# rskew/aiko_services

Measured on AMD Instinct MI355X. Metric: frames/sec (whole node) + p50 latency, ResNet-50 pipeline at 1/2/4/8 MI355X, higher is better.
Workload: dtype bf16; 1 GPU; global_batch=640, per_gpu_batch=640, parallelism=dp1, hipgraph=True, ingest=hbm, setup_frames=12, model=resnet50, pipeline=(SyntheticFrames ResNet50Classifier ClassifierTopK), gpu_lanes=2

## Files before the change

### aiko_services_amd/csrc/kernels/bneck_fused.hip

```cpp
#include <cstdlib>
#include <type_traits>

#include "conv_common.h"

namespace aiko {

namespace {

constexpr int kBnW = 56;
constexpr int kBnMid = 64;
constexpr int kBnOut = 256;
constexpr int kBnNW = 8;
constexpr int kBnTPW = 2;
constexpr int kBnTU = 8 * 64 + 8;
constexpr int kBnTB = kBnTU * 16;

struct BnParams {
  const bf16_t* x;
  const bf16_t* w1;
  const float* b1;
  const bf16_t* w2;
  const float* b2;
  const bf16_t* w3;
  const float* b3;
  bf16_t* y;
  int B, H;
  int rows_per_wg, rows_rem;
  unsigned* dbg;
  int mode;
};

__device__ __forceinline__ void bn_barrier() {
  asm volatile("s_waitcnt lgkmcnt(0)\n\ts_barrier" ::: "memory");
}

__device__ __forceinline__ void bn_vm_wait(int n) {
  switch (n) {
#define BN_W(k) case k: asm volatile("s_waitcnt vmcnt(" #k ")" ::: "memory"); break;
    BN_W(1) BN_W(2) BN_W(3) BN_W(4) BN_W(5) BN_W(6) BN_W(7) BN_W(8) BN_W(9) BN_W(10) BN_W(11) BN_W(12)
    BN_W(13) BN_W(14) BN_W(15) BN_W(16) BN_W(17) BN_W(18) BN_W(19) BN_W(20) BN_W(21) BN_W(22) BN_W(23)
    BN_W(24) BN_W(25) BN_W(26) BN_W(27) BN_W(28)
#undef BN_W
    default: asm volatile("s_waitcnt vmcnt(0)" ::: "memory"); break;
  }
}

template <int KS, int R, int D>
__device__ __forceinline__ void bn_pipeline() {
  __builtin_amdgcn_sched_group_barrier(0x100, R * D, 0);
#pragma unroll
  for (int k = 0; k < KS - D; ++k) {
    __builtin_amdgcn_sched_group_barrier(0x008, R, 0);
    __builtin_amdgcn_sched_group_barrier(0x100, R, 0);
  }
  __builtin_amdgcn_sched_group_barrier(0x008, R * D, 0);
}

__device__ __forceinline__ void bn_store16(bf16_t* p, u32x4 v) {
  asm volatile("global_store_dwordx4 %0, %1, off\n\ts_nop 1" :: "v"(p), "v"(v) : "memory");
}

template <int OFF>
__device__ __forceinline__ bf16x8 bn_ld(const unsigned char* base) {
  return *reinterpret_cast<const bf16x8*>(base + OFF);
}

__device__ __forceinline__ uint32_t bn_relu2(uint32_t v) {
  typedef short s16x2 __attribute__((ext_vector_type(2)));
  const s16x2 r = __builtin_elementwise_max(__builtin_bit_cast(s16x2, v), s16x2{0, 0});
  return __builtin_bit_cast(uint32_t, r);
}

template <int CIN>
__global__ __launch_bounds__(64 * kBnNW, 1) void bneck_fused_kernel(BnParams p) {
  constexpr bool DUAL = CIN == 64;
  constexpr int NC = CIN / 8;
  constexpr int XPU = NC + 2;
  constexpr int XU = kBnW * XPU;
  constexpr int XB = XU * 16;
  constexpr int NI = (XU + 63) / 64;
  constexpr int DQ = (NI + kBnNW - 1) / kBnNW;
  constexpr int KS1 = CIN / 32, KS2 = 9 * kBnMid / 32, K3 = DUAL ? 2 * kBnMid : kBnMid, KS3 = K3 / 32;
  constexpr int ST = 2 * kBnTPW;
  constexpr int X_BYTES = 4 * XB, T1_BYTES = 3 * kBnTB;
  constexpr int LDS_BYTES = X_BYTES + T1_BYTES + kBnTB;
  static_assert(LDS_BYTES <= 160 * 1024, "LDS");
  __shared__ __attribute__((aligned(16))) unsigned char lds[LDS_BYTES];
  unsigned char* const xr = lds;
  unsigned char* const t1r = lds + X_BYTES;
  unsigned char* const t2b = lds + X_BYTES + T1_BYTES;

  const int tid = threadIdx.x, lane = tid & 63;
  const int wv = __builtin_amdgcn_readfirstlane(tid >> 6);
  const int cg = wv & 3;
  const int pt0 = (wv >> 2) * kBnTPW;
  const int fr = lane & 15, fq = lane >> 4;

  const int lid = xcd_remap(blockIdx.x, gridDim.x);
  const int H = p.H, HV = H + 2;
  const int R0 = lid * p.rows_per_wg + min(lid, p.rows_rem);
  const int nrows = p.rows_per_wg + (lid < p.rows_rem ? 1 : 0);
  if (nrows <= 0) return;
  const int n0 = R0 / H, h0 = R0 - n0 * H;

  bf16x8 w1f[KS1], w2f[KS2], w3f[4][KS3];
#pragma unroll
  for (int ks = 0; ks < KS1; ++ks)
    w1f[ks] = *reinterpret_cast<const bf16x8*>(p.w1 + (16 * cg + fr) * CIN + 32 * ks + 8 * fq);
#pragma unroll
  for (int ks = 0; ks < KS2; ++ks)
    w2f[ks] = *reinterpret_cast<const bf16x8*>(p.w2 + (16 * cg + fr) * (9 * kBnMid) + 32 * ks + 8 * fq);
#pragma unroll
  for (int t = 0; t < 4; ++t) {
    const int row = 64 * cg + 32 * (t >> 1) + 8 * (fr >> 2) + 4 * (t & 1) + (fr & 3);
#pragma unroll
    for (int ks = 0; ks < KS3; ++ks)
      w3f[t][ks] = *reinterpret_cast<const bf16x8*>(p.w3 + row * K3 + 32 * ks + 8 * fq);
  }
  f32x4 bias1, bias2;
#pragma unroll
  for (int e = 0; e < 4; ++e) {
    bias1[e] = p.b1[16 * cg + 4 * fq + e];
    bias2[e] = p.b2[16 * cg + 4 * fq + e];
  }
  f32x4 bias3[4];
#pragma unroll
  for (int t = 0; t < 4; ++t)
#pragma unroll
    for (int e = 0; e < 4; ++e) bias3[t][e] = p.b3[64 * cg + 32 * (t >> 1) + 8 * fq + 4 * (t & 1) + e];
  bf16x8 eye[2];
#pragma unroll
  for (int tp = 0; tp < 2; ++tp)
#pragma unroll
    for (int i = 0; i < 8; ++i)
      eye[tp][i] = (fq == (fr >> 2) && i == 4 * tp + (fr & 3)) ? (bf16_t)1.0f : (bf16_t)0.0f;
  if (tid < 3) *reinterpret_cast<u32x4*>(t1r + tid * kBnTB) = u32x4{0u, 0u, 0u, 0u};
  __builtin_amdgcn_s_waitcnt(0x0f70);

  int goff[DQ];
  bool gok[DQ];
#pragma unroll
  for (int q = 0; q < DQ; ++q) {
    const int u = (wv + kBnNW * q) * 64 + lane;
    const int s = min(u / XPU, kBnW - 1);
    const int c = min(u - (u / XPU) * XPU, NC - 1);
    goff[q] = s * CIN * 2 + c * 16;
    gok[q] = u < XU && wv + kBnNW * q < NI && u - (u / XPU) * XPU < NC;
  }
  int dw = 0;
#pragma unroll
  for (int q = 0; q < DQ; ++q) dw += wv + kBnNW * q < NI ? 1 : 0;

  const int xlb = ((16 * pt0 + fr) * XPU + fq) * 16;
  const int tlb = (fq * 64 + fr + 16 * pt0) * 16;
  const int twb = ((2 * cg + (fq >> 1)) * 64 + fr + 16 * pt0) * 16 + (fq & 1) * 8;

  constexpr long XROWG = (long)kBnW * CIN * 2;
  const int nl = (R0 + nrows - 1) / H;
  const int vlast = (nl - n0) * HV + (R0 + nrows - 1 - nl * H) + 2;
  int ops = 0;
  unsigned long long marks = 0;
  int vdma = h0, dn = n0, dr = h0 - 1;
  auto dma_next = [&]() {
    const int v = vdma++;
    int m = -1;
    if (dr >= 0 && dr < H) {
      const unsigned char* src = reinterpret_cast<const unsigned char*>(p.x) + ((long)dn * H + dr) * XROWG;
      unsigned char* dst = xr + (v & 3) * XB;
#pragma unroll
      for (int q = 0; q < DQ; ++q) {
        const int j = wv + kBnNW * q;
        if (gok[q]) glds16_asm(src + goff[q], dst + j * 1024);
      }
      ops += dw;
      m = ops;
    }
    if (++dr > H) {
      dr = -1;
      ++dn;
    }
    marks = (marks << 16) | (m >= 0 ? 0x8000ull | (unsigned)(m & 0x7fff) : 0ull);
  };
  auto slot_mark = [&](int v) {
    return (unsigned)(marks >> (16 * (vdma - 1 - v))) & 0xffffu;
  };
  auto row_valid = [&](int v) { return (slot_mark(v) & 0x8000u) != 0; };
  auto wait_row = [&](int v) {
    const unsigned mk = slot_mark(v);
    if (mk & 0x8000u) bn_vm_wait(__builtin_amdgcn_readfirstlane((int)(((unsigned)ops - mk) & 0x7fffu)));
  };

  auto conv1 = [&](int k) {
    unsigned char* t1w = t1r + (k % 3) * kBnTB + twb;
    if (!row_valid(k)) {
#pragma unroll
      for (int t = 0; t < kBnTPW; ++t) *reinterpret_cast<uint2*>(t1w + (1 + 16 * t) * 16) = uint2{0u, 0u};
      return;
    }
    const unsigned char* xs = xr + (k & 3) * XB + xlb;
    f32x4 a1[kBnTPW];
#pragma unroll
    for (int ks = 0; ks < KS1; ++ks) {
      bf16x8 bf[kBnTPW];
#pragma unroll
      for (int t = 0; t < kBnTPW; ++t)
        bf[t] = *reinterpret_cast<const bf16x8*>(xs + (16 * t * XPU + 4 * ks) * 16);
#pragma unroll
      for (int t = 0; t < kBnTPW; ++t)
        a1[t] = __builtin_amdgcn_mfma_f32_16x16x32_bf16(w1f[ks], bf[t], ks == 0 ? bias1 : a1[t], 0, 0, 0);
    }
    bn_pipeline<KS1, kBnTPW, KS1 >= 4 ? 3 : 1>();
#pragma unroll
    for (int t = 0; t < kBnTPW; ++t) {
      uint2 pk{bn_relu2(pack2(a1[t][0], a1[t][1])), bn_relu2(pack2(a1[t][2], a1[t][3]))};
      if (pt0 + t == 3 && fr >= kBnW - 48) pk = uint2{0u, 0u};
      *reinterpret_cast<uint2*>(t1w + (1 + 16 * t) * 16) = pk;
    }
  };

  f32x4 a2n[kBnTPW];
  auto conv2_part = [&](int vc, auto kb, auto ke) __attribute__((always_inline)) {
    constexpr int KB = decltype(kb)::value, KE = decltype(ke)::value;
    const unsigned char* tr[3] = {t1r + ((vc - 1) % 3) * kBnTB + tlb, t1r + (vc % 3) * kBnTB + tlb,
                                  t1r + ((vc + 1) % 3) * kBnTB + tlb};
#pragma unroll
    for (int ks = KB; ks < KE; ++ks) {
      const int tap = ks >> 1, dy = tap / 3, dx = tap % 3 - 1, hk = ks & 1;
      bf16x8 bf[kBnTPW];
#pragma unroll
      for (int t = 0; t < kBnTPW; ++t)
        bf[t] = *reinterpret_cast<const bf16x8*>(tr[dy] + (1 + 256 * hk + 16 * t + dx) * 16);
#pragma unroll
      for (int t = 0; t < kBnTPW; ++t)
        a2n[t] = __builtin_amdgcn_mfma_f32_16x16x32_bf16(w2f[ks], bf[t], ks == 0 ? bias2 : a2n[t], 0, 0, 0);
    }
    bn_pipeline<KE - KB, kBnTPW, 4>();
  };
  auto conv2_store = [&]() __attribute__((always_inline)) {
    unsigned char* t2w = t2b + twb;
#pragma unroll
    for (int t = 0; t < kBnTPW; ++t) {
      const uint2 pk{bn_relu2(pack2(a2n[t][0], a2n[t][1])), bn_relu2(pack2(a2n[t][2], a2n[t][3]))};
      *reinterpret_cast<uint2*>(t2w + (1 + 16 * t) * 16) = pk;
    }
  };
  using KB0 = std::integral_constant<int, 0>;
  using KBS = std::integral_constant<int, 12>;
  using KBE = std::integral_constant<int, KS2>;

  auto conv3 = [&](int vc, int n, int r) {
    const unsigned char* xres = xr + (vc & 3) * XB + xlb;
    const unsigned char* t2r = t2b + tlb;
    bf16_t* yrow = p.y + ((long)(n * H + r) * kBnW + 16 * pt0 + fr) * kBnOut + 64 * cg + 8 * fq;
#pragma unroll
    for (int t8 = 0; t8 < kBnTPW; ++t8) {
      bf16x8 bf[KS3];
#pragma unroll
      for (int ks = 0; ks < KS3; ++ks)
        bf[ks] = ks < 2 ? *reinterpret_cast<const bf16x8*>(t2r + (1 + 256 * ks + 16 * t8) * 16)
                        : *reinterpret_cast<const bf16x8*>(xres + (16 * t8 * XPU + 4 * (ks - 2)) * 16);
      bf16x8 rv[2];
      if constexpr (!DUAL) {
#pragma unroll
        for (int h = 0; h < 2; ++h)
          rv[h] = *reinterpret_cast<const bf16x8*>(xres + (16 * t8 * XPU + 8 * cg + 4 * h) * 16);
      }
      f32x4 a3[4];
#pragma unroll
      for (int ks = 0; ks < KS3; ++ks)
#pragma unroll
        for (int t = 0; t < 4; ++t)
          a3[t] = __builtin_amdgcn_mfma_f32_16x16x32_bf16(w3f[t][ks], bf[ks], ks == 0 ? bias3[t] : a3[t], 0, 0, 0);
      if constexpr (!DUAL) {
#pragma unroll
        for (int t = 0; t < 4; ++t) a3[t] = __builtin_amdgcn_mfma_f32_16x16x32_bf16(eye[t & 1], rv[t >> 1], a3[t], 0, 0, 0);
      }
#pragma unroll
      for (int h = 0; h < 2; ++h) {
        const u32x4 ov{bn_relu2(pack2(a3[2 * h][0], a3[2 * h][1])), bn_relu2(pack2(a3[2 * h][2], a3[2 * h][3])),
                       bn_relu2(pack2(a3[2 * h + 1][0], a3[2 * h + 1][1])),
                       bn_relu2(pack2(a3[2 * h + 1][2], a3[2 * h + 1][3]))};
        if (p.mode & 128) {
          if (ov[0] == 0x7fc07fc0u && ov[1] == ov[2] && ov[3] == 1u) bn_store16(yrow, ov);
        } else if (p.mode & 256) {
          bf16_t* yr = p.y + ((long)(n * H + r) * kBnW) * kBnOut;
          bn_store16(yr + (long)(((cg * 2 + (pt0 >> 1)) * 4 + t8 * 2 + h) % 28) * 512 + lane * 8, ov);
        } else if (16 * (pt0 + t8) + fr < kBnW) {
          bn_store16(yrow + 16 * t8 * kBnOut + 32 * h, ov);
        }
      }
    }
    ops += ST;
  };

  while (vdma <= min(h0 + 3, vlast)) dma_next();
  wait_row(min(h0 + 2, vlast));
  wait_row(h0 + 1);
  wait_row(h0);
  bn_barrier();
  conv1(h0);
  conv1(h0 + 1);
  if (h0 + 2 <= vlast) conv1(h0 + 2);
  bn_barrier();

  int n = n0, r = h0, vc = h0 + 1;
  const bool stamps = p.dbg != nullptr && wv == 0;
  unsigned st[8];
  bool pre = false;
  auto stamp = [&](int i) {
    if (stamps) st[i] = (unsigned)__builtin_amdgcn_s_memtime();
  };
  for (int j = 0; j < nrows; ++j) {
    stamp(0);
    if (j > 0) {
      if (++r == H) {
        r = 0;
        ++n;
        vc += 3;
      } else {
        ++vc;
      }
    }
    while (!(p.mode & 32) && vdma <= min(vc + 3, vlast)) dma_next();
    stamp(1);
    if (j > 0 && r == 0) {
      wait_row(vc + 1);
      wait_row(vc);
      bn_barrier();
      conv1(vc);
      conv1(vc + 1);
      bn_barrier();
    }
    if (!(p.mode & 1)) {
      if (pre) conv2_part(vc, KBS{}, KBE{});
      else conv2_part(vc, KB0{}, KBE{});
      conv2_store();
    }
    stamp(2);
    if (!(p.mode & 8) && vc + 2 <= vlast) wait_row(vc + 2);
    stamp(3);
    if (!(p.mode & 16)) bn_barrier();
    stamp(4);
    const bool split = (p.mode & 3072) && j + 1 < nrows && r + 1 < H;
    if (split && (p.mode & 2048)) conv2_part(vc + 1, KB0{}, KBS{});
    if (p.mode & 512) {
      if (!(p.mode & 4)) conv3(vc, n, r);
      stamp(5);
      if (!(p.mode & 2) && vc + 2 <= vlast) conv1(vc + 2);
    } else {
      if (!(p.mode & 2) && vc + 2 <= vlast) conv1(vc + 2);
      stamp(5);
      if (!(p.mode & 4)) conv3(vc, n, r);
    }
    if (split && !(p.mode & 2048)) conv2_part(vc + 1, KB0{}, KBS{});
    pre = split;
    stamp(6);
    if (!(p.mode & 16)) bn_barrier();
    stamp(7);
    if (stamps) {
      unsigned* d = p.dbg + ((long)lid * (p.rows_per_wg + 1) + j) * 8;
      if (lane == 0) {
        bn_store16(reinterpret_cast<bf16_t*>(d), u32x4{st[0], st[1], st[2], st[3]});
        bn_store16(reinterpret_cast<bf16_t*>(d + 4), u32x4{st[4], st[5], st[6], st[7]});
      }
      ops += 2;
    }
  }
  asm volatile("s_waitcnt vmcnt(0)" ::: "memory");
}

}

}

static int bn_cu_count() {
  static int n = 0;
  if (n == 0) {
    int dev = 0;
    if (hipGetDevice(&dev) != hipSuccess ||
        hipDeviceGetAttribute(&n, hipDeviceAttributeMultiprocessorCount, dev) != hipSuccess || n <= 0)
      n = 256;
  }
  return n;
}

extern "C" int aiko_bneck_fused(const void* x, const void* w1, const float* b1, const void* w2, const float* b2,
                                const void* w3, const float* b3, void* y, int B, int H, int W, int cin, int grid,
                                unsigned* dbg, hipStream_t stream) {
  using namespace aiko;
  if (W != kBnW || (cin != 64 && cin != 256) || B <= 0 || H <= 0) return -1;
  const int R = B * H;
  int G = grid > 0 ? grid : bn_cu_count();
  G = G < R ? G : R;
  BnParams p;
  p.x = static_cast<const bf16_t*>(x);
  p.w1 = static_cast<const bf16_t*>(w1);
  p.b1 = b1;
  p.w2 = static_cast<const bf16_t*>(w2);
  p.b2 = b2;
  p.w3 = static_cast<const bf16_t*>(w3);
  p.b3 = b3;
  p.y = static_cast<bf16_t*>(y);
  p.B = B;
  p.H = H;
  p.rows_per_wg = R / G;
  p.rows_rem = R % G;
  p.dbg = dbg;
  const char* mode = getenv("AIKO_BN_MODE");
  p.mode = mode ? atoi(mode) : 1024;
  if (cin == 256)
    hipLaunchKernelGGL(bneck_fused_kernel<256>, dim3(G), dim3(64 * kBnNW), 0, stream, p);
  else
    hipLaunchKernelGGL(bneck_fused_kernel<64>, dim3(G), dim3(64 * kBnNW), 0, stream, p);
  return (int)hipGetLastError();
}
```

Before: 98750 frames/s.

## Add lean bottleneck kernel path with rotating LDS buffers and specialized interior rows

Adds a LEAN template variant of the fused bottleneck kernel, enabled by default unless debug stamps or a non-default mode are set. It uses rotating LDS slot offsets for the input and conv1 rows, and asm helpers for global-to-LDS DMA and stores with immediate offsets. It also splits the per-row loop into a boundary path and a stripped-down interior path, and overlaps the next row's conv2 prefix with the current row. The aim is to cut per-row index arithmetic, branching and waits in the inner pipeline. In exchange it adds a second large code path whose boundary handling must be exactly right.

```diff
diff --git a/aiko_services_amd/csrc/kernels/bneck_fused.hip b/aiko_services_amd/csrc/kernels/bneck_fused.hip
--- a/aiko_services_amd/csrc/kernels/bneck_fused.hip
+++ b/aiko_services_amd/csrc/kernels/bneck_fused.hip
@@ -60,6 +60,19 @@
   asm volatile("global_store_dwordx4 %0, %1, off\n\ts_nop 1" :: "v"(p), "v"(v) : "memory");
 }
 
+template <bool HALF>
+__device__ __forceinline__ void bn_store16_row(const unsigned char* row, uint32_t off, u32x4 v) {
+  if constexpr (HALF)
+    asm volatile("global_store_dwordx4 %0, %1, off offset:64\n\ts_nop 1" :: "v"(row + off), "v"(v) : "memory");
+  else
+    asm volatile("global_store_dwordx4 %0, %1, off\n\ts_nop 1" :: "v"(row + off), "v"(v) : "memory");
+}
+
+__device__ __forceinline__ void bn_glds16_row(const unsigned char* row, uint32_t off, uint32_t m0v) {
+  asm volatile("s_mov_b32 m0, %1\n\ts_nop 0\n\tglobal_load_lds_dwordx4 %0, off"
+               :: "v"(row + off), "s"(m0v) : "memory", "m0");
+}
+
 template <int OFF>
 __device__ __forceinline__ bf16x8 bn_ld(const unsigned char* base) {
   return *reinterpret_cast<const bf16x8*>(base + OFF);
@@ -71,7 +84,7 @@
   return __builtin_bit_cast(uint32_t, r);
 }
 
-template <int CIN>
+template <int CIN, bool LEAN>
 __global__ __launch_bounds__(64 * kBnNW, 1) void bneck_fused_kernel(BnParams p) {
   constexpr bool DUAL = CIN == 64;
   constexpr int NC = CIN / 8;
@@ -292,6 +305,197 @@
     }
     ops += ST;
   };
+
+  if constexpr (LEAN) {
+    static_assert(ST + DQ <= 28, "bn_vm_wait");
+    const int Rend = R0 + nrows;
+    const int nle = (Rend - 1) / H, hle = Rend - 1 - nle * H;
+    const int F0 = h0 > 0 ? R0 - 1 : R0;
+    const int F1 = hle + 1 < H ? Rend : Rend - 1;
+    const unsigned char* const xg = reinterpret_cast<const unsigned char*>(p.x);
+    const uint32_t xm0 = __builtin_amdgcn_readfirstlane(static_cast<uint32_t>(reinterpret_cast<uintptr_t>(xr))) +
+                         wv * 1024;
+    auto dma_row = [&](const unsigned char* src, uint32_t slot) {
+#pragma unroll
+      for (int q = 0; q < DQ; ++q)
+        if (gok[q]) bn_glds16_row(src, (uint32_t)goff[q], xm0 + slot + q * (kBnNW * 1024));
+    };
+    auto wait_dma = [&]() {
+      if (dw == DQ) bn_vm_wait(ST + DQ);
+      else bn_vm_wait(ST + DQ - 1);
+    };
+    auto conv1_x = [&](uint32_t xo, uint32_t to) {
+      unsigned char* t1w = t1r + to + twb;
+      const unsigned char* xs = xr + xo + xlb;
+      f32x4 a1[kBnTPW];
+#pragma unroll
+      for (int ks = 0; ks < KS1; ++ks) {
+        bf16x8 bf[kBnTPW];
+#pragma unroll
+        for (int t = 0; t < kBnTPW; ++t)
+          bf[t] = *reinterpret_cast<const bf16x8*>(xs + (16 * t * XPU + 4 * ks) * 16);
+#pragma unroll
+        for (int t = 0; t < kBnTPW; ++t)
+          a1[t] = __builtin_amdgcn_mfma_f32_16x16x32_bf16(w1f[ks], bf[t], ks == 0 ? bias1 : a1[t], 0, 0, 0);
+      }
+      bn_pipeline<KS1, kBnTPW, KS1 >= 4 ? 3 : 1>();
+#pragma unroll
+      for (int t = 0; t < kBnTPW; ++t) {
+        uint2 pk{bn_relu2(pack2(a1[t][0], a1[t][1])), bn_relu2(pack2(a1[t][2], a1[t][3]))};
+        if (pt0 + t == 3 && fr >= kBnW - 48) pk = uint2{0u, 0u};
+        *reinterpret_cast<uint2*>(t1w + (1 + 16 * t) * 16) = pk;
+      }
+    };
+    auto conv1_zero = [&](uint32_t to) {
+      unsigned char* t1w = t1r + to + twb;
+#pragma unroll
+      for (int t = 0; t < kBnTPW; ++t) *reinterpret_cast<uint2*>(t1w + (1 + 16 * t) * 16) = uint2{0u, 0u};
+    };
+    auto conv2_rows = [&](uint32_t o0, uint32_t o1, uint32_t o2, auto kb, auto ke) __attribute__((always_inline)) {
+      constexpr int KB = decltype(kb)::value, KE = decltype(ke)::value;
+      const unsigned char* tr[3] = {t1r + o0 + tlb, t1r + o1 + tlb, t1r + o2 + tlb};
+#pragma unroll
+      for (int ks = KB; ks < KE; ++ks) {
+        const int tap = ks >> 1, dy = tap / 3, dx = tap % 3 - 1, hk = ks & 1;
+        bf16x8 bf[kBnTPW];
+#pragma unroll
+        for (int t = 0; t < kBnTPW; ++t)
+          bf[t] = *reinterpret_cast<const bf16x8*>(tr[dy] + (1 + 256 * hk + 16 * t + dx) * 16);
+#pragma unroll
+        for (int t = 0; t < kBnTPW; ++t)
+          a2n[t] = __builtin_amdgcn_mfma_f32_16x16x32_bf16(w2f[ks], bf[t], ks == 0 ? bias2 : a2n[t], 0, 0, 0);
+      }
+      bn_pipeline<KE - KB, kBnTPW, 4>();
+    };
+    const uint32_t yoff = ((16 * pt0 + fr) * kBnOut + 64 * cg + 8 * fq) * 2;
+    auto conv3_row = [&](uint32_t xo, const unsigned char* yrow) {
+      const unsigned char* xres = xr + xo + xlb;
+      const unsigned char* t2r = t2b + tlb;
+#pragma unroll
+      for (int t8 = 0; t8 < kBnTPW; ++t8) {
+        bf16x8 bf[KS3];
+#pragma unroll
+        for (int ks = 0; ks < KS3; ++ks)
+          bf[ks] = ks < 2 ? *reinterpret_cast<const bf16x8*>(t2r + (1 + 256 * ks + 16 * t8) * 16)
+                          : *reinterpret_cast<const bf16x8*>(xres + (16 * t8 * XPU + 4 * (ks - 2)) * 16);
+        bf16x8 rv[2];
+        if constexpr (!DUAL) {
+#pragma unroll
+          for (int h = 0; h < 2; ++h)
+            rv[h] = *reinterpret_cast<const bf16x8*>(xres + (16 * t8 * XPU + 8 * cg + 4 * h) * 16);
+        }
+        f32x4 a3[4];
+#pragma unroll
+        for (int ks = 0; ks < KS3; ++ks)
+#pragma unroll
+          for (int t = 0; t < 4; ++t)
+            a3[t] = __builtin_amdgcn_mfma_f32_16x16x32_bf16(w3f[t][ks], bf[ks], ks == 0 ? bias3[t] : a3[t], 0, 0, 0);
+        if constexpr (!DUAL) {
+#pragma unroll
+          for (int t = 0; t < 4; ++t) a3[t] = __builtin_amdgcn_mfma_f32_16x16x32_bf16(eye[t & 1], rv[t >> 1], a3[t], 0, 0, 0);
+        }
+        const uint32_t yo = yoff + t8 * (16 * kBnOut * 2);
+        const bool live = 16 * (pt0 + t8) + fr < kBnW;
+        const u32x4 o0{bn_relu2(pack2(a3[0][0], a3[0][1])), bn_relu2(pack2(a3[0][2], a3[0][3])),
+                       bn_relu2(pack2(a3[1][0], a3[1][1])), bn_relu2(pack2(a3[1][2], a3[1][3]))};
+        if (live) bn_store16_row<false>(yrow, yo, o0);
+        const u32x4 o1{bn_relu2(pack2(a3[2][0], a3[2][1])), bn_relu2(pack2(a3[2][2], a3[2][3])),
+                       bn_relu2(pack2(a3[3][0], a3[3][1])), bn_relu2(pack2(a3[3][2], a3[3][3]))};
+        if (live) bn_store16_row<true>(yrow, yo, o1);
+      }
+    };
+
+    const uint32_t s0 = h0 > 0 ? 1u : 0u;
+    uint32_t X0 = s0 * XB, X1 = (s0 + 1) * XB, X2 = (s0 + 2) * XB, X3 = ((s0 + 3) & 3u) * XB;
+    uint32_t T0 = 0, T1 = kBnTB, T2 = 2 * kBnTB;
+    int f = R0;
+    const unsigned char* src = xg + (long)(R0 + 3) * XROWG;
+    const unsigned char* yp = reinterpret_cast<const unsigned char*>(p.y) + (long)R0 * (kBnW * kBnOut * 2);
+    bool pre = false;
+    auto advance = [&]() {
+      ++f;
+      src += XROWG;
+      yp += kBnW * kBnOut * 2;
+      const uint32_t x0 = X0;
+      X0 = X1, X1 = X2, X2 = X3, X3 = x0;
+    };
+    auto rotate_t1 = [&]() {
+      const uint32_t t0 = T0;
+      T0 = T1, T1 = T2, T2 = t0;
+    };
+
+    auto row_general = [&](int r, int rb, int xe, bool boundary) {
+      const bool dma = f + 3 <= F1;
+      if (dma) dma_row(src, X3);
+      if (boundary) {
+        conv1_x(X0, T1);
+        if (1 <= xe) conv1_x(X1, T2);
+        else conv1_zero(T2);
+        bn_barrier();
+      }
+      if (pre) conv2_rows(T0, T1, T2, KBS{}, KBE{});
+      else conv2_rows(T0, T1, T2, KB0{}, KBE{});
+      conv2_store();
+      if (dma) wait_dma();
+      else bn_vm_wait(ST);
+      bn_barrier();
+      if (r + 2 <= xe) conv1_x(X2, T0);
+      else conv1_zero(T0);
+      conv3_row(X0, yp);
+      pre = r + 1 < rb;
+      if (pre) {
+        rotate_t1();
+        conv2_rows(T0, T1, T2, KB0{}, KBS{});
+      }
+      bn_barrier();
+      advance();
+    };
+    auto row_interior = [&]() {
+      dma_row(src, X3);
+      conv2_rows(T0, T1, T2, KBS{}, KBE{});
+      conv2_store();
+      wait_dma();
+      bn_barrier();
+      conv1_x(X2, T0);
+      conv3_row(X0, yp);
+      rotate_t1();
+      conv2_rows(T0, T1, T2, KB0{}, KBS{});
+      bn_barrier();
+      advance();
+    };
+
+    int r = h0, rem = nrows;
+    {
+      const unsigned char* s = xg + (long)F0 * XROWG;
+      const int npro = min(R0 + 2, F1) - F0 + 1;
+      for (int k = 0; k < npro; ++k, s += XROWG) dma_row(s, k * XB);
+      asm volatile("s_waitcnt vmcnt(0)" ::: "memory");
+      bn_barrier();
+      if (h0 > 0) conv1_x(X3, T0);
+      else conv1_zero(T0);
+      conv1_x(X0, T1);
+      if (h0 + 1 <= min(min(H, h0 + nrows), H - 1)) conv1_x(X1, T2);
+      else conv1_zero(T2);
+      bn_barrier();
+    }
+    bool boundary = false;
+    while (rem > 0) {
+      const int rb = min(H, r + rem);
+      const int xe = min(rb, H - 1);
+      const int rint = r + rem <= H ? xe - 2 : xe - 1;
+      rem -= rb - r;
+      for (;;) {
+        row_general(r, rb, xe, boundary);
+        boundary = false;
+        if (++r >= rb) break;
+        for (; r < rint; ++r) row_interior();
+      }
+      r = 0;
+      boundary = true;
+    }
+    asm volatile("s_waitcnt vmcnt(0)" ::: "memory");
+    return;
+  }
 
   while (vdma <= min(h0 + 3, vlast)) dma_next();
   wait_row(min(h0 + 2, vlast));
@@ -408,9 +612,10 @@
   p.dbg = dbg;
   const char* mode = getenv("AIKO_BN_MODE");
   p.mode = mode ? atoi(mode) : 1024;
-  if (cin == 256)
-    hipLaunchKernelGGL(bneck_fused_kernel<256>, dim3(G), dim3(64 * kBnNW), 0, stream, p);
-  else
-    hipLaunchKernelGGL(bneck_fused_kernel<64>, dim3(G), dim3(64 * kBnNW), 0, stream, p);
+  const char* lean = getenv("AIKO_BN_LEAN");
+  const bool use_lean = dbg == nullptr && p.mode == 1024 && !(lean && atoi(lean) == 0);
+  auto* kernel = cin == 256 ? (use_lean ? bneck_fused_kernel<256, true> : bneck_fused_kernel<256, false>)
+                            : (use_lean ? bneck_fused_kernel<64, true> : bneck_fused_kernel<64, false>);
+  hipLaunchKernelGGL(kernel, dim3(G), dim3(64 * kBnNW), 0, stream, p);
   return (int)hipGetLastError();
 }
```

New measurement: 100,200 frames/s (median of 6 runs). 1.4% higher.
